# mks0601/ExAvatar_RELEASE

Hardware: NVIDIA H100
Metric: avatar train-step frames/sec (fwd+bwd raster) (higher is better)
Workload: dtype f32

## Files before the change

exavatar_release_b200/csrc/binning.cu:

```cuda
#include <cstdlib>

#include "common.cuh"

namespace b2r {

__global__ void __launch_bounds__(256) scatter_kernel(const B2RScene sc, const Ctx cx, const int first_row) {
  const int i = first_row + blockIdx.x * blockDim.x + threadIdx.x;
  int4 aux = make_int4(0, 0, 0, 0);
  float4 g0 = make_float4(0.f, 0.f, 0.f, 0.f), g1 = g0;
  uint32_t depth_bits = 0u;
  if (i < sc.P) {
    aux = cx.aux[i];
    if (aux.z > 0) {
      const int area = ((aux.y & 0xffff) - (aux.x & 0xffff)) * ((aux.y >> 16) - (aux.x >> 16));
      depth_bits = __float_as_uint(cx.geom[i].g1.z);
      if (area > 32) {
        g0 = reinterpret_cast<const float4*>(cx.geom + i)[0];
        g1 = reinterpret_cast<const float4*>(cx.geom + i)[1];
      }
    }
  }
  const uint64_t cap = cx.dup_capacity;
  const int gx = cx.gx;
  uint32_t* cursor = cx.tile_cursor;
// ... 25 lines not shown
      const int area = ((aux.y & 0xffff) - (aux.x & 0xffff)) * ((aux.y >> 16) - (aux.x >> 16));
      depth_bits = __float_as_uint(cx.geom[i].g1.z);
      if (area > 32) {
        g0 = reinterpret_cast<const float4*>(cx.geom + i)[0];
        g1 = reinterpret_cast<const float4*>(cx.geom + i)[1];
      }
    }
  }
  const int gx = cx.gx;
  const bool no_cull = (sc.flags & B2R_FLAG_NO_TILE_CULL) != 0;
  const int x0 = aux.x & 0xffff, y0 = aux.x >> 16, x1 = aux.y & 0xffff, y1 = aux.y >> 16;
  const uint32_t kept = (uint32_t)aux.w;
  warp_replay_kept_tiles(aux.z > 0, x0, y0, x1, y1, kept, g0.x, g0.y, g0.z, g0.w, g1.x, g1.w, 0u, 0u, no_cull, sc.width,
                         sc.height, gx, s_cnt, [](uint32_t, int, uint32_t, uint32_t) {});
  __syncthreads();
  for (int t = threadIdx.x; t < cx.tiles; t += blockDim.x) {
    const uint32_t c = s_cnt[t];
    if (c) {
      s_base[t] = atomicAdd(cx.tile_cursor + t, c);
      s_cnt[t] = 0u;
    }
  }
  __syncthreads();
  const uint64_t cap = cx.dup_capacity;
  uint2* keys = cx.keys;
  warp_replay_kept_tiles(aux.z > 0, x0, y0, x1, y1, kept, g0.x, g0.y, g0.z, g0.w, g1.x, g1.w, depth_bits, (uint32_t)i,
                         no_cull, sc.width, sc.height, gx, s_cnt, [&](uint32_t rank, int t, uint32_t d, uint32_t id) {
                           const uint32_t pos = s_base[t] + rank;
                           if (pos < cap) keys[pos] = make_uint2(d, id);
                         });
}


__device__ __forceinline__ unsigned match_digit(const uint32_t d, const bool valid) {
  unsigned peers = __ballot_sync(0xffffffffu, valid);
#pragma unroll
  for (int bit = 0; bit < 8; bit++) {
    const bool on = (d >> bit) & 1u;
    const unsigned b = __ballot_sync(0xffffffffu, on);
    peers &= on ? b : ~b;
  }
  return valid ? peers : 0u;
}

template <int CAP, int THREADS>
struct RadixSmem {
  static constexpr int W = THREADS / 32;
  static constexpr size_t bytes = (size_t)CAP * 12 + (size_t)W * 256 * 2 + 64;
};

template <int CAP, int THREADS, bool PAIRS = false>
__device__ __forceinline__ void radix_sort_tile(const uint2* src, uint32_t* dst, const int n, unsigned char* smem_raw,
                                                uint32_t* maxid) {
  constexpr int W = THREADS / 32;
  constexpr int ROWS = CAP / (W * 32);
  static_assert(CAP % (W * 32) == 0, "a warp's share must be whole rows");
  uint32_t* keyA = reinterpret_cast<uint32_t*>(smem_raw);
  uint32_t* keyB = keyA + CAP;
  uint16_t* idxA = reinterpret_cast<uint16_t*>(keyB + CAP);
  uint16_t* idxB = idxA + CAP;
  uint16_t* hist = idxB + CAP;
  uint32_t* misc = reinterpret_cast<uint32_t*>(hist + W * 256);
  const int tid = threadIdx.x, lane = tid & 31, warp = tid >> 5;

  if (tid == 0) { misc[0] = 0u; misc[1] = 0xffffffffu; }
  __syncthreads();
  uint32_t vor = 0u, vand = 0xffffffffu;
  for (int i = tid; i < n; i += THREADS) {
    const uint32_t k = src[i].x;
    keyA[i] = k;
    idxA[i] = (uint16_t)i;
    vor |= k;
    vand &= k;
  }
  vor = __reduce_or_sync(0xffffffffu, vor);
  vand = __reduce_and_sync(0xffffffffu, vand);
  if (lane == 0) { atomicOr(&misc[0], vor); atomicAnd(&misc[1], vand); }
  __syncthreads();
  const uint32_t differ = misc[0] ^ misc[1];

  const int chunk = (((n + W - 1) / W) + 31) & ~31;
  const int c_begin = min(warp * chunk, n), c_end = min(c_begin + chunk, n);
  uint32_t* kin = keyA; uint32_t* kout = keyB;
  uint16_t* iin = idxA; uint16_t* iout = idxB;
  for (int pass = 0; pass < 4; pass++) {
    const int shift = 8 * pass;
    if (((differ >> shift) & 0xffu) == 0u) continue;
    for (int i = tid; i < W * 256; i += THREADS) hist[i] = 0;
    __syncthreads();
    uint16_t* myhist = hist + warp * 256;
    unsigned row_peers[ROWS];
#pragma unroll
    for (int r = 0; r < ROWS; r++) {
      const int base = c_begin + 32 * r;
      row_peers[r] = 0u;
      if (base < c_end) {
        const int i = base + lane;
        const bool valid = i < c_end;
        const uint32_t d = valid ? ((kin[i] >> shift) & 0xffu) : (256u + lane);
        const unsigned peers = match_digit(d, valid);
        row_peers[r] = peers;
        if (valid && (peers & ((1u << lane) - 1u)) == 0u) myhist[d] = (uint16_t)(myhist[d] + __popc(peers));
        __syncwarp();
      }
    }
    __syncthreads();
    constexpr int DPT = THREADS >= 256 ? 1 : 256 / THREADS;
    constexpr int SCAN_THREADS = 256 / DPT;
    uint32_t tot[DPT];
    uint32_t total = 0;
    if (tid < SCAN_THREADS) {
#pragma unroll
      for (int r = 0; r < DPT; r++) {
        const int d = tid * DPT + r;
        uint32_t run = 0;
        for (int w = 0; w < W; w++) {
          const uint32_t t = hist[w * 256 + d];
          hist[w * 256 + d] = (uint16_t)run;
          run += t;
        }
        tot[r] = run;
        total += run;
      }
    }
    uint32_t incl = total;
#pragma unroll
    for (int o = 1; o < 32; o <<= 1) {
      const uint32_t v = __shfl_up_sync(0xffffffffu, incl, o);
      if (lane >= o) incl += v;
    }
    if (tid < SCAN_THREADS && lane == 31) misc[2 + warp] = incl;
    __syncthreads();
    if (tid < SCAN_THREADS) {
      uint32_t base = incl - total;
      for (int w = 0; w < warp; w++) base += misc[2 + w];
#pragma unroll
      for (int r = 0; r < DPT; r++) {
        const int d = tid * DPT + r;
        for (int w = 0; w < W; w++) hist[w * 256 + d] = (uint16_t)(hist[w * 256 + d] + base);
        base += tot[r];
      }
    }
    __syncthreads();
#pragma unroll
    for (int r = 0; r < ROWS; r++) {
      const int base = c_begin + 32 * r;
      if (base < c_end) {
        const int i = base + lane;
        const bool valid = i < c_end;
        const uint32_t k = valid ? kin[i] : 0u;
        const uint32_t d = (k >> shift) & 0xffu;
        const unsigned peers = row_peers[r];
        const unsigned below = peers & ((1u << lane) - 1u);
        uint32_t start = 0;
        if (valid && below == 0u) {
          start = myhist[d];
          myhist[d] = (uint16_t)(start + __popc(peers));
        }
        start = __shfl_sync(0xffffffffu, start, valid ? __ffs(peers) - 1 : lane);
        if (valid) {
          const uint32_t o = start + __popc(below);
          kout[o] = k;
          iout[o] = iin[i];
        }
        __syncwarp();
      }
    }
    __syncthreads();
    { uint32_t* t = kin; kin = kout; kout = t; }
    { uint16_t* t = iin; iin = iout; iout = t; }
  }
  uint32_t* ids = kout;
  uint32_t vmax = 0u;
  for (int i = tid; i < n; i += THREADS) {
    const uint32_t id = src[iin[i]].y;
    ids[i] = id;
    vmax = max(vmax, id);
  }
  vmax = __reduce_max_sync(0xffffffffu, vmax);
  if (lane == 0 && vmax) atomicMax(maxid, vmax);
  __syncthreads();
  for (;;) {
    int changed = 0;
#pragma unroll
    for (int phase = 0; phase < 2; phase++) {
      for (int i = 2 * tid + phase; i + 1 < n; i += 2 * THREADS) {
        if (kin[i] == kin[i + 1]) {
          const uint32_t a = ids[i], b = ids[i + 1];
          if (a > b) { ids[i] = b; ids[i + 1] = a; changed = 1; }
        }
      }
      __syncthreads();
    }
    if (!__syncthreads_or(changed)) break;
  }
  if (PAIRS) {
    uint2* out = const_cast<uint2*>(src);
    for (int i = tid; i < n; i += THREADS) out[i] = make_uint2(kin[i], ids[i]);
  } else {
    for (int i = tid; i < n; i += THREADS) dst[i] = ids[i];
  }
  __syncthreads();
}

constexpr int WSORT_CAP = 1 << SORT_CTA_SHIFT;
constexpr size_t WSORT_BYTES = (size_t)WSORT_CAP * 12 + 256 * 2;

__device__ __forceinline__ void warp_sort_tile(const uint2* __restrict__ src, uint32_t* __restrict__ dst, const int n,
                                               unsigned char* smem_warp, uint32_t* __restrict__ maxid) {
  const int lane = threadIdx.x & 31;
  const unsigned below_mask = (1u << lane) - 1u;
  if (n <= 0) return;
  if (n <= 32) {
    const uint2 kv = lane < n ? src[lane] : make_uint2(0xffffffffu, 0xffffffffu);
    const uint32_t m = __reduce_max_sync(0xffffffffu, lane < n ? kv.y : 0u);
    if (lane == 0) *maxid = m;
    const unsigned long long me = ((unsigned long long)kv.x << 32) | kv.y;
    int rank = 0;
    for (int j = 0; j < n; j++) {
      const unsigned long long o = __shfl_sync(0xffffffffu, me, j);
      rank += (o < me) ? 1 : 0;
    }
    if (lane < n) dst[rank] = kv.y;
    return;
  }
  uint32_t* keyA = reinterpret_cast<uint32_t*>(smem_warp);
  uint32_t* keyB = keyA + WSORT_CAP;
  uint16_t* idxA = reinterpret_cast<uint16_t*>(keyB + WSORT_CAP);
  uint16_t* idxB = idxA + WSORT_CAP;
  uint16_t* hist = idxB + WSORT_CAP;
  uint32_t vor = 0u, vand = 0xffffffffu;
  for (int i = lane; i < n; i += 32) {
    const uint32_t k = src[i].x;
    keyA[i] = k;
    idxA[i] = (uint16_t)i;
    vor |= k;
    vand &= k;
  }
  const uint32_t differ = __reduce_or_sync(0xffffffffu, vor) ^ __reduce_and_sync(0xffffffffu, vand);
  __syncwarp();
  uint32_t* kin = keyA; uint32_t* kout = keyB;
  uint16_t* iin = idxA; uint16_t* iout = idxB;
  for (int pass = 0; pass < 4; pass++) {
    const int shift = 8 * pass;
    if (((differ >> shift) & 0xffu) == 0u) continue;
    reinterpret_cast<uint4*>(hist)[lane] = make_uint4(0u, 0u, 0u, 0u);
    __syncwarp();
    constexpr int CACHED = 8;
    unsigned row_peers[CACHED];
#pragma unroll
    for (int r = 0; r < CACHED; r++) {
      const int base = 32 * r;
      row_peers[r] = 0u;
      if (base < n) {
        const int i = base + lane;
        const bool valid = i < n;
        const uint32_t d = valid ? ((kin[i] >> shift) & 0xffu) : (256u + lane);
        const unsigned peers = match_digit(d, valid);
        row_peers[r] = peers;
        if (valid && (peers & below_mask) == 0u) hist[d] = (uint16_t)(hist[d] + __popc(peers));
        __syncwarp();
      }
    }
    for (int base = 32 * CACHED; base < n; base += 32) {
// ... 16 lines not shown
    uint32_t run = incl - total;
#pragma unroll
    for (int r = 0; r < 8; r++) { hist[8 * lane + r] = (uint16_t)run; run += c[r]; }
    __syncwarp();
    auto place_row = [&](const int base, const bool cached, const unsigned cached_peers) {
        const int i = base + lane;
        const bool valid = i < n;
        const uint32_t k = valid ? kin[i] : 0u;
        const uint32_t d = valid ? ((k >> shift) & 0xffu) : (256u + lane);
        const unsigned peers = cached ? cached_peers : match_digit(d, valid);
        const unsigned below = peers & below_mask;
        uint32_t start = 0;
        if (valid && below == 0u) {
          start = hist[d];
          hist[d] = (uint16_t)(start + __popc(peers));
        }
        start = __shfl_sync(0xffffffffu, start, valid ? __ffs(peers) - 1 : lane);
        if (valid) {
          const uint32_t o = start + __popc(below);
          kout[o] = k;
          iout[o] = iin[i];
        }
        __syncwarp();
    };
#pragma unroll
    for (int r = 0; r < CACHED; r++)
      if (32 * r < n) place_row(32 * r, true, row_peers[r]);
    for (int base = 32 * CACHED; base < n; base += 32) place_row(base, false, 0u);
    { uint32_t* t = kin; kin = kout; kout = t; }
    { uint16_t* t = iin; iin = iout; iout = t; }
  }
  uint32_t* ids = kout;
  uint32_t vmax = 0u;
  for (int i = lane; i < n; i += 32) {
    const uint32_t id = src[iin[i]].y;
    ids[i] = id;
    vmax = max(vmax, id);
  }
  vmax = __reduce_max_sync(0xffffffffu, vmax);
  if (lane == 0) *maxid = vmax;
  __syncwarp();
  for (;;) {
    bool changed = false;
#pragma unroll
    for (int phase = 0; phase < 2; phase++) {
      for (int i = 2 * lane + phase; i + 1 < n; i += 64) {
        if (kin[i] == kin[i + 1]) {
          const uint32_t a = ids[i], b = ids[i + 1];
          if (a > b) { ids[i] = b; ids[i + 1] = a; changed = true; }
        }
      }
      __syncwarp();
    }
    if (!__any_sync(0xffffffffu, changed)) break;
  }
  for (int i = lane; i < n; i += 32) dst[i] = ids[i];
  __syncwarp();
}

template <int CAP, int THREADS>
__global__ void __launch_bounds__(THREADS) sort_mixed_kernel(const Ctx cx) {
  extern __shared__ __align__(16) unsigned char smem_raw[];
  B2R_TRACE_BEGIN();
  const unsigned long long cls = cx.status->reserved[0];
  const int n_large = (int)(cls & 0xffffffffull), n_ge512 = (int)(cls >> 32);
  const int n_chunks = (int)cx.status->reserved[1];
  const int n_cta = n_ge512 - n_large;
  const int n_warp_items = (cx.tiles - n_ge512 + (THREADS / 32) - 1) / (THREADS / 32);
  const int items = n_chunks + n_cta + n_warp_items;
  int last_n = 0;
  for (int b = blockIdx.x; b < items; b += gridDim.x) {
    if (b < n_chunks) {
      int lo = 0, hi = n_large - 1;
      while (lo < hi) {
        const int mid = (lo + hi + 1) >> 1;
        if ((int)cx.chunk_start[mid] <= b) lo = mid; else hi = mid - 1;
      }
      const uint32_t tile = cx.tile_order[lo];
      const uint2 r = cx.ranges[tile];
      const int off = (b - (int)cx.chunk_start[lo]) * SORT_CHUNK;
      const int len = min(SORT_CHUNK, sort_length(cx, (int)tile, r) - off);
      if (len > 1) radix_sort_tile<CAP, THREADS, true>(cx.keys + r.x + off, nullptr, len, smem_raw, cx.tile_maxid + tile);
      else if (len == 1 && threadIdx.x == 0) atomicMax(cx.tile_maxid + tile, cx.keys[r.x + off].y);
      last_n = len;
    } else if (b < n_chunks + n_cta) {
      const uint32_t tile = cx.tile_order[n_large + (b - n_chunks)];
      const uint2 r = cx.ranges[tile];
      const int n = sort_length(cx, (int)tile, r);
      const uint2* src = cx.keys + r.x;
      uint32_t* dst = cx.dup_ids + r.x;
      if (n > 32) {
        radix_sort_tile<CAP, THREADS>(src, dst, n, smem_raw, cx.tile_maxid + tile);
      } else {
        if (threadIdx.x < 32) warp_sort_tile(src, dst, n, smem_raw, cx.tile_maxid + tile);
// ... 105 lines not shown
    launch_tile_scan(quiet, st);
  }
  if (sc.P > 0) {
    ProfScope p(K_SCATTER, st);
    const size_t smem = (size_t)cx.tiles * 8;
    if (cx.tiles <= 2048) {
      cudaFuncSetAttribute(scatter_agg_kernel, cudaFuncAttributeMaxDynamicSharedMemorySize, 96 * 1024);
      launch_k(scatter_agg_kernel, (sc.P + 255) / 256, 256, smem, st, true, sc, cx, 0);
    } else {
      launch_k(scatter_kernel, (sc.P + 255) / 256, 256, 0, st, true, sc, cx, 0);
    }
  }
  launch_sort(cx, st);
  return check_launch();
}

void launch_sort(const Ctx& cx, cudaStream_t st) {
  const int sms = device_sm_count();
  constexpr int ST = 256;
  constexpr size_t cta_bytes = RadixSmem<SORT_SMALL, ST>::bytes, warp_bytes = (ST / 32) * WSORT_BYTES;
  constexpr size_t small_bytes = cta_bytes > warp_bytes ? cta_bytes : warp_bytes;
  cudaFuncSetAttribute(sort_mixed_kernel<SORT_SMALL, ST>, cudaFuncAttributeMaxDynamicSharedMemorySize, (int)small_bytes);
  {
    ProfScope p(K_SORT_SMALL, st);
    launch_k(sort_mixed_kernel<SORT_SMALL, ST>, cx.tiles, ST, small_bytes, st, true, cx);
  }
  {
    ProfScope p(K_SORT_LARGE, st);
    launch_k(merge_chunks_kernel, 2 * sms, 256, 0, st, true, cx);
  }
}


__global__ void __launch_bounds__(256) split_prepare_kernel(const Ctx cx, const Ctx base, const int split,
                                                            int32_t* __restrict__ radii) {
  const int tid = threadIdx.x;
  const float4* gsrc = reinterpret_cast<const float4*>(base.geom);
  float4* gdst = reinterpret_cast<float4*>(cx.geom);
  for (size_t k = (size_t)blockIdx.x * 256 + tid; k < (size_t)split * 3; k += (size_t)gridDim.x * 256) gdst[k] = gsrc[k];
  for (int k = blockIdx.x * 256 + tid; k < split; k += gridDim.x * 256) radii[k] = base.aux[k].z;
  for (int t = blockIdx.x; t < cx.tiles; t += gridDim.x) {
    const uint32_t own = cx.tile_count[t];
    uint32_t s = 0;
    if (own) {
      const uint2 rb = base.ranges[t];
      for (uint32_t k = rb.x; k < rb.y; k += 256)
        s += (uint32_t)__syncthreads_count(k + tid < rb.y && base.dup_ids[k + tid] < (uint32_t)split);
    }
    if (tid == 0) {
      cx.sort_len[t] = own;
      cx.tile_count[t] = own + s;
    }
    __syncthreads();
  }
}

constexpr int SPLIT_CHUNK = 2048;
constexpr int SPLIT_PER = 8;
__global__ void __launch_bounds__(256) split_merge_kernel(const Ctx cx, const Ctx base, const uint32_t* __restrict__ own_ids,
                                                          const int split) {
  __shared__ uint2 other[SPLIT_CHUNK];
  __shared__ uint32_t wtot[8];
  const int tid = threadIdx.x, lane = tid & 31, warp = tid >> 5;
  const uint32_t tile = cx.tile_order[blockIdx.x];
  const uint2 r = cx.ranges[tile];
  const int n = (int)(r.y - r.x);
  if (n == 0) return;
  const int n_own = sort_length(cx, (int)tile, r);
  uint2* keys = cx.keys + r.x;
  for (int i = tid; i < n_own; i += 256) {
    const uint32_t id = own_ids[r.x + i];
    keys[i] = make_uint2(__float_as_uint(cx.geom[id].g1.z), id);
  }
  const uint2 rb = base.ranges[tile];
  int n_base = 0;
  for (uint32_t k0 = rb.x; k0 < rb.y; k0 += 256) {
    const uint32_t k = k0 + tid;
    const uint32_t id = k < rb.y ? base.dup_ids[k] : 0xffffffffu;
    const bool take = id < (uint32_t)split;
    const unsigned b = __ballot_sync(0xffffffffu, take);
    if (lane == 0) wtot[warp] = __popc(b);
    __syncthreads();
    int off = n_base, tot = 0;
    for (int w = 0; w < 8; w++) {
      off += w < warp ? (int)wtot[w] : 0;
      tot += (int)wtot[w];
    }
    off += __popc(b & ((1u << lane) - 1u));
    if (take && n_own + off < n) keys[n_own + off] = make_uint2(__float_as_uint(cx.geom[id].g1.z), id);
    n_base += tot;
    __syncthreads();
  }
  __syncthreads();
  if (n_own + n_base != n) {
    for (int i = tid; i < n; i += 256) cx.dup_ids[r.x + i] = keys[i].y;
    return;
  }
  for (int side = 0; side < 2; side++) {
    const uint2* mine = side ? keys + n_own : keys;
    const uint2* oth = side ? keys : keys + n_own;
    const int n_mine = side ? n_base : n_own, n_oth = side ? n_own : n_base;
    for (int x0 = 0; x0 < n_mine; x0 += 256 * SPLIT_PER) {
      unsigned long long key[SPLIT_PER];
      int rank[SPLIT_PER];
#pragma unroll
      for (int j = 0; j < SPLIT_PER; j++) {
        const int i = x0 + j * 256 + tid;
        const uint2 v = i < n_mine ? mine[i] : make_uint2(0u, 0u);
        key[j] = ((unsigned long long)v.x << 32) | v.y;
        rank[j] = i;
      }
      for (int c0 = 0; c0 < n_oth; c0 += SPLIT_CHUNK) {
        const int len2 = min(SPLIT_CHUNK, n_oth - c0);
        __syncthreads();
        for (int i = tid; i < len2; i += 256) other[i] = oth[c0 + i];
        __syncthreads();
#pragma unroll
        for (int j = 0; j < SPLIT_PER; j++) {
          int l = 0;
          for (int step = SPLIT_CHUNK; step >= 1; step >>= 1) {
            const int probe = l + step;
            if (probe <= len2) {
              const uint2 v = other[probe - 1];
              if ((((unsigned long long)v.x << 32) | v.y) < key[j]) l = probe;
            }
          }
          rank[j] += l;
        }
      }
#pragma unroll
      for (int j = 0; j < SPLIT_PER; j++)
        if (x0 + j * 256 + tid < n_mine) cx.dup_ids[r.x + rank[j]] = (uint32_t)(key[j] & 0xffffffffull);
    }
  }
}

int launch_binning_split(const B2RScene& sc, const Ctx& cx_in, const Ctx& base, uint32_t* own_ids, const int first_row,
                         int32_t* radii, cudaStream_t st) {
  const Ctx& cx = cx_in;
  {
    ProfScope p(K_MISC, st);
    launch_k(split_prepare_kernel, cx.tiles, 256, 0, st, true, cx, base, first_row, radii);
  }
  launch_tile_scan(cx, st, cx.dup_capacity > 0 ? 1 : 0);
  if (sc.P > first_row) {
    ProfScope p(K_SCATTER, st);
    const unsigned grid = (unsigned)((sc.P - first_row + 255) / 256);
    if (cx.tiles <= 2048) {
      cudaFuncSetAttribute(scatter_agg_kernel, cudaFuncAttributeMaxDynamicSharedMemorySize, 96 * 1024);
      launch_k(scatter_agg_kernel, grid, 256, (size_t)cx.tiles * 8, st, true, sc, cx, first_row);
    } else {
      launch_k(scatter_kernel, grid, 256, 0, st, true, sc, cx, first_row);
    }
  }
  Ctx own = cx;
  own.dup_ids = own_ids;
  launch_sort(own, st);
  {
    ProfScope p(K_SORT_LARGE, st);
    launch_k(split_merge_kernel, cx.tiles, 256, 0, st, true, cx, base, own_ids, first_row);
  }
  return check_launch();
}

}
// ... 7 lines not shown
```

exavatar_release_b200/csrc/composite_bwd4.cu:

```cuda
#include "common.cuh"

namespace b2r {

constexpr int B4_THREADS = 64;
constexpr int B4_BATCH = 64;
#ifndef B4_QUEUE_DEPTH
#define B4_QUEUE_DEPTH 16
#endif
#ifndef B4_MIN_BLOCKS
#define B4_MIN_BLOCKS 10
#endif
constexpr int B4_QUEUE = B4_QUEUE_DEPTH;

struct B4Stage {
  float4 a[B4_BATCH];
  float4 b[B4_BATCH];
  float4 c[B4_BATCH];
};
constexpr int B4_GROUP = 4;
constexpr int B4_CQ = 32 + B4_GROUP;
struct B4Compact {
  float4 r[3][B4_CQ];
};
static_assert(B4_QUEUE % B4_GROUP == 0, "phase B runs when whole groups fill the transposition queue");

__device__ __forceinline__ float rcp_approx4(float x) {
  float y;
  asm("rcp.approx.ftz.f32 %0, %1;" : "=f"(y) : "f"(x));
  return y;
}

struct B4Smem {
  B4Stage stage[2];
  B4Compact compact[2];
  float2 tb[2][B4_QUEUE][33];
  float4 qm0[2][B4_QUEUE];
  float4 qm1[2][B4_QUEUE];
  float4 gpix[2][32];
  int warp_max_s[2];
};

template <bool HAS_DA>
__device__ __forceinline__ void bwd4_item(const B2RScene& sc, const Ctx& cx, const B2RBackwardArgs& args,
                                          float* __restrict__ gacc, B4Smem& sm, const int t_pos, const int seg,
                                          const int quad, const int n_multi) {
  B4Stage (&stage)[2] = sm.stage;
  B4Compact (&compact)[2] = sm.compact;
  float2 (&tb)[2][B4_QUEUE][33] = sm.tb;
  float4 (&qm0)[2][B4_QUEUE] = sm.qm0;
  float4 (&qm1)[2][B4_QUEUE] = sm.qm1;
  float4 (&gpix)[2][32] = sm.gpix;
  int (&warp_max_s)[2] = sm.warp_max_s;
  B2R_TRACE_BEGIN();
  const bool multi = t_pos < n_multi;
  const int tile = (int)cx.tile_order[t_pos];
  if (cx.skip_below && cx.tile_maxid[tile] < cx.skip_below) return;
  const int tx = tile % cx.gx, ty = tile / cx.gx;
  const int lane = threadIdx.x & 31, warp = threadIdx.x >> 5;
  const int W = sc.width, H = sc.height;
  const int wx0 = tx * TILE + (quad & 1) * 8, wy0 = ty * TILE + (quad >> 1) * 8 + warp * 4;
  if (wx0 >= W || ty * TILE + (quad >> 1) * 8 >= H) return;
  const int px = wx0 + (lane & 7), py = wy0 + (lane >> 3);
  const bool inside = px < W && py < H;
  const float pxf = (float)px, pyf = (float)py;
  const float rx0 = (float)wx0, ry0 = (float)wy0;
  const float rx1 = fminf((float)(wx0 + 7), (float)(W - 1)), ry1 = fminf((float)(wy0 + 3), (float)(H - 1));
  const size_t N = (size_t)W * H;
  const size_t pix = (size_t)py * W + px;

  const uint2 range = cx.ranges[tile];
  const int n = (int)(range.y - range.x);
  const int lo = multi ? seg * SEG : 0;
  const int hi = multi ? min(n, lo + SEG) : n;
  const uint32_t* ids = cx.dup_ids + range.x + lo;

  const int my_n = inside ? (int)cx.n_contrib[pix] : 0;
  const int my_hi = min(my_n, hi) - lo;
  const bool cont = my_n > hi;
  const float T_final = inside ? cx.final_T[pix] : 0.f;
  const float g_r = inside ? __ldg(args.dL_dcolor + pix) : 0.f;
  const float g_g = inside ? __ldg(args.dL_dcolor + N + pix) : 0.f;
  const float g_b = inside ? __ldg(args.dL_dcolor + 2 * N + pix) : 0.f;
  float g_d = 0.f, g_a = 0.f;
// ... 3 lines not shown
  }
  const float* bgp = cx.bg ? cx.bg : sc.bg;
  const float Tfb = T_final * (__ldg(bgp) * g_r + __ldg(bgp + 1) * g_g + __ldg(bgp + 2) * g_b);
  gpix[warp][lane] = make_float4(g_r, g_g, g_b, g_d);

  const int warp_n = __reduce_max_sync(0xffffffffu, max(my_hi, 0));
  if (lane == 0) warp_max_s[warp] = warp_n;
  __syncthreads();
  const int nmax = max(warp_max_s[0], warp_max_s[1]);
  if (nmax == 0) {
    B2R_TRACE_END(0);
    return;
  }
  const int nb = (nmax + B4_BATCH - 1) / B4_BATCH;

  float T = T_final, B = 0.f;
  if (cont) {
    const int pit = (py - ty * TILE) * TILE + (px - tx * TILE);
    const int nrec = (n + SEG - 1) / SEG;
    const float* rec = cx.ckpt + (size_t)(cx.seg_start[t_pos] + seg) * CK_REC_FLOATS;
    const float* fin = cx.ckpt + (size_t)(cx.seg_start[t_pos] + nrec - 1) * CK_REC_FLOATS;
    const float4 c = __ldg(reinterpret_cast<const float4*>(rec) + pit);
    const float4 f = __ldg(reinterpret_cast<const float4*>(fin) + pit);
    float num = (f.y - c.y) * g_r + (f.z - c.z) * g_g + (f.w - c.w) * g_b;
    if (HAS_DA) {
      const float2 c2 = __ldg(reinterpret_cast<const float2*>(rec + CK_PLANE0) + pit);
      const float2 f2 = __ldg(reinterpret_cast<const float2*>(fin + CK_PLANE0) + pit);
      num += (f2.x - c2.x) * g_d + (f2.y - c2.y) * g_a;
    }
    T = c.x;
    B = __fdividef(num, c.x);
  }
  float la = 0.f, olm = 1.f, lv = 0.f;
  int qpos = 0;
  B4Compact& cw = compact[warp];
  const bool lane0 = lane == 0;
  const unsigned lanes_above = 0xfffffffeu << lane;
  const uint32_t first_grad = args.first_row;

  auto drain = [&](const int count) {
    constexpr int SHARE = 32 / B4_QUEUE;
    constexpr int ROWS = 4 / SHARE;
    static_assert(B4_QUEUE == 8 || B4_QUEUE == 16 || B4_QUEUE == 32, "queue depth");
    __syncwarp();
    const int h = lane & (B4_QUEUE - 1), part = lane / B4_QUEUE;
    const bool live = h < count;
    float Sx = 0.f, Sy = 0.f, Sxx = 0.f, Sxy = 0.f, Syy = 0.f, Sq = 0.f, Sr = 0.f, Sg = 0.f, Sb = 0.f, Sd = 0.f;
    float4 m0 = make_float4(0.f, 0.f, 0.f, 0.f), m1 = make_float4(0.f, 1.f, 0.f, 0.f);
    if (live) {
      m0 = qm0[warp][h];
      m1 = qm1[warp][h];
      const float mx = m0.x - rx0, my = m0.y - ry0;
      float dxs[8];
#pragma unroll
      for (int c = 0; c < 8; c++) dxs[c] = mx - (float)c;
#pragma unroll
      for (int r = 0; r < ROWS; r++) {
        const float dy = my - (float)(part * ROWS + r);
        float Rq = 0.f, Rx = 0.f, Rxx = 0.f;
#pragma unroll
        for (int c = 0; c < 8; c++) {
          const int p = (part * ROWS + r) * 8 + c;
          const float2 t = tb[warp][h][p];
          const float4 g = gpix[warp][p];
          const float hx = t.x * dxs[c];
          Rq += t.x;
          Rx += hx;
          Rxx = fmaf(hx, dxs[c], Rxx);
          Sr = fmaf(t.y, g.x, Sr);
          Sg = fmaf(t.y, g.y, Sg);
          Sb = fmaf(t.y, g.z, Sb);
          if (HAS_DA) Sd = fmaf(t.y, g.w, Sd);
        }
        const float hy = Rq * dy;
        Sq += Rq;
        Sx += Rx;
        Sxx += Rxx;
        Sy += hy;
        Syy = fmaf(hy, dy, Syy);
        Sxy = fmaf(Rx, dy, Sxy);
      }
    }
#pragma unroll
    for (int o = B4_QUEUE; o < 32; o <<= 1) {
      Sx += __shfl_xor_sync(0xffffffffu, Sx, o);
      Sy += __shfl_xor_sync(0xffffffffu, Sy, o);
      Sxx += __shfl_xor_sync(0xffffffffu, Sxx, o);
      Sxy += __shfl_xor_sync(0xffffffffu, Sxy, o);
      Syy += __shfl_xor_sync(0xffffffffu, Syy, o);
      Sq += __shfl_xor_sync(0xffffffffu, Sq, o);
      Sr += __shfl_xor_sync(0xffffffffu, Sr, o);
      Sg += __shfl_xor_sync(0xffffffffu, Sg, o);
      Sb += __shfl_xor_sync(0xffffffffu, Sb, o);
      if (HAS_DA) Sd += __shfl_xor_sync(0xffffffffu, Sd, o);
    }
    const uint32_t gid = __float_as_uint(m1.z) & 0x1fffffffu;
    if (live && part == 0 && gid >= first_grad) {
      float* dst = gacc + (size_t)gid * 12;
      red_add_v4(dst, 2.f * m0.z * Sx + m0.w * Sy, 2.f * m1.x * Sy + m0.w * Sx, Sxx, Sxy);
      red_add_v4(dst + 4, Syy, __fdividef(Sq, m1.y), Sd, 0.f);
      red_add_v4(dst + 8, Sr, Sg, Sb, 0.f);
    }
    __syncwarp();
  };

  const uint32_t id_begin = cx.id_begin, id_span = cx.id_span;
  uint32_t next_id = 0u;
  auto prefetch = [&](int b) {
    const int idx = b * B4_BATCH + threadIdx.x;
    next_id = idx < nmax ? __ldg(ids + idx) : 0u;
  };
  auto issue = [&](int b) {
    B4Stage& s = stage[b & 1];
    const int idx = b * B4_BATCH + threadIdx.x;
    if (idx < nmax) {
      const uint32_t id = next_id;
      if (id - id_begin < id_span) {
        const float4* src = reinterpret_cast<const float4*>(cx.geom + id);
        cp_async16(&s.a[threadIdx.x], src);
        cp_async16(&s.b[threadIdx.x], src + 1);
        cp_async16(&s.c[threadIdx.x], src + 2);
      } else {
        s.a[threadIdx.x] = make_float4(0.f, 0.f, -1.f, 0.f);
        s.b[threadIdx.x] = make_float4(-1.f, 0.f, 0.f, INFINITY);
      }
    }
    cp_async_commit();
  };

  auto replay_group = [&](const int k) {
    float araw[B4_GROUP], vv[B4_GROUP];
    bool valid[B4_GROUP];
#pragma unroll
    for (int u = 0; u < B4_GROUP; u++) {
      const float4 a = cw.r[0][k + u], bb = cw.r[1][k + u], col = cw.r[2][k + u];
      const float dx = a.x - pxf, dy = a.y - pyf;
      const float p2 = a.z * dx * dx + bb.x * dy * dy + a.w * dx * dy;
      araw[u] = bb.y * ex2_approx(p2);
      valid[u] = (__float_as_int(bb.w) < my_hi) && (p2 <= 0.f) && (araw[u] >= K_ALPHA_MIN);
      float v = fmaf(col.z, g_b, fmaf(col.y, g_g, col.x * g_r));
      if (HAS_DA) v += fmaf(bb.z, g_d, g_a);
      vv[u] = v;
      if (lane0) {
        qm0[warp][qpos + u] = a;
        qm1[warp][qpos + u] = make_float4(bb.x, bb.y, col.w, 0.f);
      }
    }
#pragma unroll
    for (int u = 0; u < B4_GROUP; u++) {
      const float ae = valid[u] ? fminf(K_ALPHA_MAX, araw[u]) : 0.f;
      const float om = 1.f - ae;
      const float rcp = rcp_approx4(om);
      const float Tn = T * rcp;
      B = fmaf(la, lv, olm * B);
      const float dLda = fmaf(vv[u] - B, Tn, -Tfb * rcp);
      la = ae; olm = om; lv = vv[u]; T = Tn;
      tb[warp][qpos + u][lane] = make_float2(valid[u] ? araw[u] * dLda : 0.f, ae * Tn);
    }
    qpos += B4_GROUP;
    if (qpos == B4_QUEUE) {
      drain(B4_QUEUE);
      qpos = 0;
    }
  };

  int head = 0, fill = 0;
  prefetch(nb - 1);
  issue(nb - 1);
  if (nb > 1) prefetch(nb - 2);
  for (int b = nb - 1; b >= 0; b--) {
    cp_async_wait<0>();
    __syncthreads();
    if (b > 0) {
      issue(b - 1);
      if (b > 1) prefetch(b - 2);
    }
    const int count = min(B4_BATCH, nmax - b * B4_BATCH);
    const B4Stage& s = stage[b & 1];
    if (warp_n <= b * B4_BATCH) continue;
    for (int c0 = ((count - 1) >> 5) << 5; c0 >= 0; c0 -= 32) {
      const int idx = c0 + lane;
      const int pos = b * B4_BATCH + idx;
      bool hit = false;
      float4 a, bb;
      if (idx < count && pos < warp_n) {
        a = s.a[idx];
        bb = s.b[idx];
        hit = !(region_max_p2(a.x, a.y, a.z, a.w, bb.x, rx0, ry0, rx1, ry1) < bb.w);
      }
      const unsigned mask = __ballot_sync(0xffffffffu, hit);
      if (mask == 0u) continue;
      if (hit) {
        int slot = head + fill + __popc(mask & lanes_above);
        slot -= slot >= B4_CQ ? B4_CQ : 0;
        cw.r[0][slot] = a;
        cw.r[1][slot] = make_float4(bb.x, bb.y, bb.z, __int_as_float(pos));
        cw.r[2][slot] = s.c[idx];
      }
      fill += __popc(mask);
      __syncwarp();
      for (; fill >= B4_GROUP; fill -= B4_GROUP) {
        replay_group(head);
        head = head + B4_GROUP == B4_CQ ? 0 : head + B4_GROUP;
      }
      __syncwarp();
    }
  }
  if (fill > 0) {
    if (lane >= fill && lane < B4_GROUP) {
      cw.r[0][head + lane] = make_float4(0.f, 0.f, 0.f, 0.f);
      cw.r[1][head + lane] = make_float4(0.f, 1.f, 0.f, __int_as_float(0x7fffffff));
      cw.r[2][head + lane] = make_float4(0.f, 0.f, 0.f, 0.f);
    }
    __syncwarp();
    replay_group(head);
  }
  if (qpos > 0) drain(qpos);
  if (threadIdx.x == 0) atomicAdd(reinterpret_cast<unsigned long long*>(&cx.status->consumed_bwd), (unsigned long long)nmax);
  B2R_TRACE_END(nmax);
}

template <bool HAS_DA>
__global__ void __launch_bounds__(B4_THREADS, B4_MIN_BLOCKS) composite_bwd4_kernel(const B2RScene sc, const Ctx cx,
                                                                    const B2RBackwardArgs args, float* __restrict__ gacc) {
  __shared__ B4Smem sm;
  const int n_multi = cx.ckpt ? (int)cx.classes[CLS_N_MULTI] : 0;
  const int total_segs = cx.ckpt ? (int)cx.classes[CLS_TOTAL_SEGS] : 0;
  const int items = 4 * (total_segs + (cx.tiles - n_multi));
  for (int item = blockIdx.x; item < items; item += gridDim.x) {
    const int s_item = item >> 2;
    int t_pos, seg;
    if (s_item < total_segs) {
      const uint2 e = cx.seg_table[s_item];
      t_pos = (int)e.x;
      seg = (int)e.y;
    } else {
      t_pos = n_multi + (s_item - total_segs);
      seg = 0;
    }
    bwd4_item<HAS_DA>(sc, cx, args, gacc, sm, t_pos, seg, item & 3, n_multi);
    __syncthreads();
  }
}

int launch_composite_bwd(const B2RScene& sc, const Ctx& cx, const B2RBackwardArgs& a, float* gacc, cudaStream_t st) {
  if (!(a.flags & B2R_BWD_SCRATCH_ZEROED)) cudaMemsetAsync(gacc, 0, (size_t)(sc.P > 0 ? sc.P : 1) * 12 * sizeof(float), st);
  const uint64_t extra = cx.ckpt ? cx.dup_capacity / SEG : 0;
  const uint64_t bound = 4ull * ((uint64_t)cx.tiles + extra);
  const uint64_t cap = (uint64_t)device_sm_count() * B4_MIN_BLOCKS * 4;
  const unsigned grid = (unsigned)(bound < cap ? bound : cap);
  ProfScope p(K_COMPOSITE_BWD, st);
  if (a.dL_ddepth || a.dL_dalpha)
    launch_k(composite_bwd4_kernel<true>, grid, B4_THREADS, 0, st, false, sc, cx, a, gacc);
  else
    launch_k(composite_bwd4_kernel<false>, grid, B4_THREADS, 0, st, false, sc, cx, a, gacc);
  return check_launch();
}

}

#ifdef B2R_CTA_TRACE
extern "C" int b2r_debug_trace_bwd(unsigned long long* buf) {
// ... 4 lines not shown
```

Baseline: 1904.

## Use min-offset adaptive-width radix passes and merge-path split merge

The block radix sort now takes the min/max key range, subtracts the minimum, and sorts the span in as few passes as possible with up to 10-bit digits. The histogram scan is packed as four u16 counters per thread. The split merge replaces the per-element binary search against shared-memory chunks with a merge-path partition, so each thread merges its own output slice. Gather loops are batched by SPLIT_PER for memory-level parallelism, and the sort kernel gets a min-blocks launch bound. The trade-offs are a larger histogram in shared memory, which may lower occupancy, and a serial per-thread merge loop.

```diff
diff --git a/exavatar_release_b200/csrc/binning.cu b/exavatar_release_b200/csrc/binning.cu
--- a/exavatar_release_b200/csrc/binning.cu
+++ b/exavatar_release_b200/csrc/binning.cu
@@ -81,21 +81,27 @@
 }
 
 
-__device__ __forceinline__ unsigned match_digit(const uint32_t d, const bool valid) {
+template <int MAX_BITS = 8>
+__device__ __forceinline__ unsigned match_digit(const uint32_t d, const bool valid, const int bits = MAX_BITS) {
   unsigned peers = __ballot_sync(0xffffffffu, valid);
 #pragma unroll
-  for (int bit = 0; bit < 8; bit++) {
-    const bool on = (d >> bit) & 1u;
-    const unsigned b = __ballot_sync(0xffffffffu, on);
-    peers &= on ? b : ~b;
+  for (int bit = 0; bit < MAX_BITS; bit++) {
+    if (bit < bits) {
+      const bool on = (d >> bit) & 1u;
+      const unsigned b = __ballot_sync(0xffffffffu, on);
+      peers &= on ? b : ~b;
+    }
   }
   return valid ? peers : 0u;
 }
+
+constexpr int RADIX_BITS = 10;
+constexpr int RADIX_BINS = 1 << RADIX_BITS;
 
 template <int CAP, int THREADS>
 struct RadixSmem {
   static constexpr int W = THREADS / 32;
-  static constexpr size_t bytes = (size_t)CAP * 12 + (size_t)W * 256 * 2 + 64;
+  static constexpr size_t bytes = (size_t)CAP * 12 + (size_t)W * RADIX_BINS * 2 + 64;
 };
 
 template <int CAP, int THREADS, bool PAIRS = false>
@@ -109,35 +115,42 @@
   uint16_t* idxA = reinterpret_cast<uint16_t*>(keyB + CAP);
   uint16_t* idxB = idxA + CAP;
   uint16_t* hist = idxB + CAP;
-  uint32_t* misc = reinterpret_cast<uint32_t*>(hist + W * 256);
+  uint32_t* misc = reinterpret_cast<uint32_t*>(hist + W * RADIX_BINS);
   const int tid = threadIdx.x, lane = tid & 31, warp = tid >> 5;
 
-  if (tid == 0) { misc[0] = 0u; misc[1] = 0xffffffffu; }
-  __syncthreads();
-  uint32_t vor = 0u, vand = 0xffffffffu;
+  if (tid == 0) { misc[0] = 0xffffffffu; misc[1] = 0u; }
+  __syncthreads();
+  uint32_t kmin_t = 0xffffffffu, kmax_t = 0u;
+#pragma unroll 4
   for (int i = tid; i < n; i += THREADS) {
     const uint32_t k = src[i].x;
     keyA[i] = k;
     idxA[i] = (uint16_t)i;
-    vor |= k;
-    vand &= k;
-  }
-  vor = __reduce_or_sync(0xffffffffu, vor);
-  vand = __reduce_and_sync(0xffffffffu, vand);
-  if (lane == 0) { atomicOr(&misc[0], vor); atomicAnd(&misc[1], vand); }
-  __syncthreads();
-  const uint32_t differ = misc[0] ^ misc[1];
+    kmin_t = min(kmin_t, k);
+    kmax_t = max(kmax_t, k);
+  }
+  kmin_t = __reduce_min_sync(0xffffffffu, kmin_t);
+  kmax_t = __reduce_max_sync(0xffffffffu, kmax_t);
+  if (lane == 0) { atomicMin(&misc[0], kmin_t); atomicMax(&misc[1], kmax_t); }
+  __syncthreads();
+  const uint32_t kmin = misc[0];
+  const int span = 32 - __clz(misc[1] - kmin);
+  const int passes = (span + RADIX_BITS - 1) / RADIX_BITS;
+  const int bits = passes ? (span + passes - 1) / passes : 0;
+  const uint32_t mask = (1u << bits) - 1u;
 
   const int chunk = (((n + W - 1) / W) + 31) & ~31;
   const int c_begin = min(warp * chunk, n), c_end = min(c_begin + chunk, n);
   uint32_t* kin = keyA; uint32_t* kout = keyB;
   uint16_t* iin = idxA; uint16_t* iout = idxB;
-  for (int pass = 0; pass < 4; pass++) {
-    const int shift = 8 * pass;
-    if (((differ >> shift) & 0xffu) == 0u) continue;
-    for (int i = tid; i < W * 256; i += THREADS) hist[i] = 0;
+  for (int pass = 0; pass < passes; pass++) {
+    const int shift = bits * pass;
+    const int zshift = max(bits - 3, 0);
+    for (int i = tid; i < (W << zshift); i += THREADS)
+      reinterpret_cast<uint4*>(hist + (i >> zshift) * RADIX_BINS)[i & ((1 << zshift) - 1)] = make_uint4(0u, 0u, 0u, 0u);
+    const bool scans = 4 * tid < (1 << bits);
     __syncthreads();
-    uint16_t* myhist = hist + warp * 256;
+    uint16_t* myhist = hist + warp * RADIX_BINS;
     unsigned row_peers[ROWS];
 #pragma unroll
     for (int r = 0; r < ROWS; r++) {
@@ -146,48 +159,44 @@
       if (base < c_end) {
         const int i = base + lane;
         const bool valid = i < c_end;
-        const uint32_t d = valid ? ((kin[i] >> shift) & 0xffu) : (256u + lane);
-        const unsigned peers = match_digit(d, valid);
+        const uint32_t d = valid ? ((kin[i] - kmin) >> shift) & mask : 0u;
+        const unsigned peers = match_digit<RADIX_BITS>(d, valid, bits);
         row_peers[r] = peers;
         if (valid && (peers & ((1u << lane) - 1u)) == 0u) myhist[d] = (uint16_t)(myhist[d] + __popc(peers));
         __syncwarp();
       }
     }
     __syncthreads();
-    constexpr int DPT = THREADS >= 256 ? 1 : 256 / THREADS;
-    constexpr int SCAN_THREADS = 256 / DPT;
-    uint32_t tot[DPT];
-    uint32_t total = 0;
-    if (tid < SCAN_THREADS) {
-#pragma unroll
-      for (int r = 0; r < DPT; r++) {
-        const int d = tid * DPT + r;
-        uint32_t run = 0;
-        for (int w = 0; w < W; w++) {
-          const uint32_t t = hist[w * 256 + d];
-          hist[w * 256 + d] = (uint16_t)run;
-          run += t;
-        }
-        tot[r] = run;
-        total += run;
-      }
-    }
+    static_assert(RADIX_BINS == 4 * THREADS && CAP < 65536, "four u16 counters per thread and warp");
+    uint2* hist4 = reinterpret_cast<uint2*>(hist) + tid;
+    uint2 run = make_uint2(0u, 0u);
+    if (scans) {
+#pragma unroll
+      for (int w = 0; w < W; w++) {
+        const uint2 c = hist4[w * THREADS];
+        hist4[w * THREADS] = run;
+        run.x += c.x;
+        run.y += c.y;
+      }
+    }
+    const uint32_t t0 = run.x & 0xffffu, t1 = run.x >> 16, t2 = run.y & 0xffffu;
+    const uint32_t total = t0 + t1 + t2 + (run.y >> 16);
     uint32_t incl = total;
 #pragma unroll
     for (int o = 1; o < 32; o <<= 1) {
       const uint32_t v = __shfl_up_sync(0xffffffffu, incl, o);
       if (lane >= o) incl += v;
     }
-    if (tid < SCAN_THREADS && lane == 31) misc[2 + warp] = incl;
+    if (lane == 31) misc[2 + warp] = incl;
     __syncthreads();
-    if (tid < SCAN_THREADS) {
+    if (scans) {
       uint32_t base = incl - total;
       for (int w = 0; w < warp; w++) base += misc[2 + w];
-#pragma unroll
-      for (int r = 0; r < DPT; r++) {
-        const int d = tid * DPT + r;
-        for (int w = 0; w < W; w++) hist[w * 256 + d] = (uint16_t)(hist[w * 256 + d] + base);
-        base += tot[r];
+      const uint2 off = make_uint2(base | ((base + t0) << 16), (base + t0 + t1) | ((base + t0 + t1 + t2) << 16));
+#pragma unroll
+      for (int w = 0; w < W; w++) {
+        const uint2 c = hist4[w * THREADS];
+        hist4[w * THREADS] = make_uint2(c.x + off.x, c.y + off.y);
       }
     }
     __syncthreads();
@@ -198,7 +207,7 @@
         const int i = base + lane;
         const bool valid = i < c_end;
         const uint32_t k = valid ? kin[i] : 0u;
-        const uint32_t d = (k >> shift) & 0xffu;
+        const uint32_t d = ((k - kmin) >> shift) & mask;
         const unsigned peers = row_peers[r];
         const unsigned below = peers & ((1u << lane) - 1u);
         uint32_t start = 0;
@@ -221,6 +230,7 @@
   }
   uint32_t* ids = kout;
   uint32_t vmax = 0u;
+#pragma unroll 4
   for (int i = tid; i < n; i += THREADS) {
     const uint32_t id = src[iin[i]].y;
     ids[i] = id;
@@ -279,6 +289,7 @@
   uint16_t* idxB = idxA + WSORT_CAP;
   uint16_t* hist = idxB + WSORT_CAP;
   uint32_t vor = 0u, vand = 0xffffffffu;
+#pragma unroll 4
   for (int i = lane; i < n; i += 32) {
     const uint32_t k = src[i].x;
     keyA[i] = k;
@@ -361,6 +372,7 @@
   }
   uint32_t* ids = kout;
   uint32_t vmax = 0u;
+#pragma unroll 4
   for (int i = lane; i < n; i += 32) {
     const uint32_t id = src[iin[i]].y;
     ids[i] = id;
@@ -388,7 +400,7 @@
 }
 
 template <int CAP, int THREADS>
-__global__ void __launch_bounds__(THREADS) sort_mixed_kernel(const Ctx cx) {
+__global__ void __launch_bounds__(THREADS, 4) sort_mixed_kernel(const Ctx cx) {
   extern __shared__ __align__(16) unsigned char smem_raw[];
   B2R_TRACE_BEGIN();
   const unsigned long long cls = cx.status->reserved[0];
@@ -560,6 +572,8 @@
 }
 
 
+constexpr int SPLIT_PER = 8;
+
 __global__ void __launch_bounds__(256) split_prepare_kernel(const Ctx cx, const Ctx base, const int split,
                                                             int32_t* __restrict__ radii) {
   const int tid = threadIdx.x;
@@ -567,13 +581,25 @@
   float4* gdst = reinterpret_cast<float4*>(cx.geom);
   for (size_t k = (size_t)blockIdx.x * 256 + tid; k < (size_t)split * 3; k += (size_t)gridDim.x * 256) gdst[k] = gsrc[k];
   for (int k = blockIdx.x * 256 + tid; k < split; k += gridDim.x * 256) radii[k] = base.aux[k].z;
+  __shared__ uint32_t wsum[8];
   for (int t = blockIdx.x; t < cx.tiles; t += gridDim.x) {
     const uint32_t own = cx.tile_count[t];
     uint32_t s = 0;
     if (own) {
       const uint2 rb = base.ranges[t];
-      for (uint32_t k = rb.x; k < rb.y; k += 256)
-        s += (uint32_t)__syncthreads_count(k + tid < rb.y && base.dup_ids[k + tid] < (uint32_t)split);
+      uint32_t c = 0;
+      for (uint32_t k0 = rb.x; k0 < rb.y; k0 += 256 * SPLIT_PER) {
+#pragma unroll
+        for (int j = 0; j < SPLIT_PER; j++) {
+          const uint32_t k = k0 + j * 256 + tid;
+          c += (k < rb.y && base.dup_ids[k] < (uint32_t)split) ? 1u : 0u;
+        }
+      }
+      c = __reduce_add_sync(0xffffffffu, c);
+      if ((tid & 31) == 0) wsum[tid >> 5] = c;
+      __syncthreads();
+#pragma unroll
+      for (int w = 0; w < 8; w++) s += wsum[w];
     }
     if (tid == 0) {
       cx.sort_len[t] = own;
@@ -583,11 +609,8 @@
   }
 }
 
-constexpr int SPLIT_CHUNK = 2048;
-constexpr int SPLIT_PER = 8;
 __global__ void __launch_bounds__(256) split_merge_kernel(const Ctx cx, const Ctx base, const uint32_t* __restrict__ own_ids,
                                                           const int split) {
-  __shared__ uint2 other[SPLIT_CHUNK];
   __shared__ uint32_t wtot[8];
   const int tid = threadIdx.x, lane = tid & 31, warp = tid >> 5;
   const uint32_t tile = cx.tile_order[blockIdx.x];
@@ -596,26 +619,54 @@
   if (n == 0) return;
   const int n_own = sort_length(cx, (int)tile, r);
   uint2* keys = cx.keys + r.x;
-  for (int i = tid; i < n_own; i += 256) {
-    const uint32_t id = own_ids[r.x + i];
-    keys[i] = make_uint2(__float_as_uint(cx.geom[id].g1.z), id);
+  for (int i0 = 0; i0 < n_own; i0 += 256 * SPLIT_PER) {
+    uint32_t id[SPLIT_PER];
+    float z[SPLIT_PER];
+#pragma unroll
+    for (int j = 0; j < SPLIT_PER; j++) {
+      const int i = i0 + j * 256 + tid;
+      id[j] = i < n_own ? own_ids[r.x + i] : 0u;
+    }
+#pragma unroll
+    for (int j = 0; j < SPLIT_PER; j++) z[j] = i0 + j * 256 + tid < n_own ? cx.geom[id[j]].g1.z : 0.f;
+#pragma unroll
+    for (int j = 0; j < SPLIT_PER; j++) {
+      const int i = i0 + j * 256 + tid;
+      if (i < n_own) keys[i] = make_uint2(__float_as_uint(z[j]), id[j]);
+    }
   }
   const uint2 rb = base.ranges[tile];
   int n_base = 0;
-  for (uint32_t k0 = rb.x; k0 < rb.y; k0 += 256) {
-    const uint32_t k = k0 + tid;
-    const uint32_t id = k < rb.y ? base.dup_ids[k] : 0xffffffffu;
-    const bool take = id < (uint32_t)split;
-    const unsigned b = __ballot_sync(0xffffffffu, take);
-    if (lane == 0) wtot[warp] = __popc(b);
+  for (uint32_t k0 = rb.x; k0 < rb.y; k0 += 256 * SPLIT_PER) {
+    uint32_t id[SPLIT_PER];
+    unsigned b[SPLIT_PER];
+    int wcount = 0;
+#pragma unroll
+    for (int j = 0; j < SPLIT_PER; j++) {
+      const uint32_t k = k0 + (warp * SPLIT_PER + j) * 32 + lane;
+      id[j] = k < rb.y ? base.dup_ids[k] : 0xffffffffu;
+    }
+#pragma unroll
+    for (int j = 0; j < SPLIT_PER; j++) {
+      b[j] = __ballot_sync(0xffffffffu, id[j] < (uint32_t)split);
+      wcount += __popc(b[j]);
+    }
+    if (lane == 0) wtot[warp] = wcount;
     __syncthreads();
     int off = n_base, tot = 0;
     for (int w = 0; w < 8; w++) {
       off += w < warp ? (int)wtot[w] : 0;
       tot += (int)wtot[w];
     }
-    off += __popc(b & ((1u << lane) - 1u));
-    if (take && n_own + off < n) keys[n_own + off] = make_uint2(__float_as_uint(cx.geom[id].g1.z), id);
+    float z[SPLIT_PER];
+#pragma unroll
+    for (int j = 0; j < SPLIT_PER; j++) z[j] = id[j] < (uint32_t)split ? cx.geom[id[j]].g1.z : 0.f;
+#pragma unroll
+    for (int j = 0; j < SPLIT_PER; j++) {
+      const int o = off + __popc(b[j] & ((1u << lane) - 1u));
+      if (id[j] < (uint32_t)split && n_own + o < n) keys[n_own + o] = make_uint2(__float_as_uint(z[j]), id[j]);
+      off += __popc(b[j]);
+    }
     n_base += tot;
     __syncthreads();
   }
@@ -624,41 +675,26 @@
     for (int i = tid; i < n; i += 256) cx.dup_ids[r.x + i] = keys[i].y;
     return;
   }
-  for (int side = 0; side < 2; side++) {
-    const uint2* mine = side ? keys + n_own : keys;
-    const uint2* oth = side ? keys : keys + n_own;
-    const int n_mine = side ? n_base : n_own, n_oth = side ? n_own : n_base;
-    for (int x0 = 0; x0 < n_mine; x0 += 256 * SPLIT_PER) {
-      unsigned long long key[SPLIT_PER];
-      int rank[SPLIT_PER];
-#pragma unroll
-      for (int j = 0; j < SPLIT_PER; j++) {
-        const int i = x0 + j * 256 + tid;
-        const uint2 v = i < n_mine ? mine[i] : make_uint2(0u, 0u);
-        key[j] = ((unsigned long long)v.x << 32) | v.y;
-        rank[j] = i;
-      }
-      for (int c0 = 0; c0 < n_oth; c0 += SPLIT_CHUNK) {
-        const int len2 = min(SPLIT_CHUNK, n_oth - c0);
-        __syncthreads();
-        for (int i = tid; i < len2; i += 256) other[i] = oth[c0 + i];
-        __syncthreads();
-#pragma unroll
-        for (int j = 0; j < SPLIT_PER; j++) {
-          int l = 0;
-          for (int step = SPLIT_CHUNK; step >= 1; step >>= 1) {
-            const int probe = l + step;
-            if (probe <= len2) {
-              const uint2 v = other[probe - 1];
-              if ((((unsigned long long)v.x << 32) | v.y) < key[j]) l = probe;
-            }
-          }
-          rank[j] += l;
-        }
-      }
-#pragma unroll
-      for (int j = 0; j < SPLIT_PER; j++)
-        if (x0 + j * 256 + tid < n_mine) cx.dup_ids[r.x + rank[j]] = (uint32_t)(key[j] & 0xffffffffull);
+  const uint2* own = keys;
+  const uint2* oth = keys + n_own;
+  const int d0 = (int)(((long long)n * tid) / 256), d1 = (int)(((long long)n * (tid + 1)) / 256);
+  if (d0 == d1) return;
+  auto key64 = [](const uint2 v) { return ((unsigned long long)v.x << 32) | v.y; };
+  int lo = max(0, d0 - n_base), hi = min(d0, n_own);
+  while (lo < hi) {
+    const int mid = (lo + hi) >> 1;
+    if (key64(own[mid]) < key64(oth[d0 - mid - 1])) lo = mid + 1; else hi = mid;
+  }
+  int i = lo, j = d0 - lo;
+  unsigned long long a = i < n_own ? key64(own[i]) : ~0ull, c = j < n_base ? key64(oth[j]) : ~0ull;
+  uint32_t* out = cx.dup_ids + r.x;
+  for (int d = d0; d < d1; d++) {
+    if (a < c) {
+      out[d] = (uint32_t)a;
+      a = ++i < n_own ? key64(own[i]) : ~0ull;
+    } else {
+      out[d] = (uint32_t)c;
+      c = ++j < n_base ? key64(oth[j]) : ~0ull;
     }
   }
 }
```

Result: no change. 1902 (median of 6 runs) (-0.1%).

## Read drain metadata from compact queue, skip drains with no gradient rows

Applied to the files above, without the earlier changes.

Removes the separate per-warp metadata queues (qm0/qm1) written by lane 0 during replay. Drain now reads Gaussian parameters directly from the compaction ring, whose size grows to 32+queue depth so that drains never wrap. Drain exits early when no entry in the batch needs a gradient (gid < first_row), and accumulator initialisation is folded into the first term. It also adds an optional half-batch staging mode where two threads split the three cp.async loads per entry, and re-reads class counts inside the item loop. The cost is a larger compact buffer and reliance on the ring-alignment invariants.

```diff
diff --git a/exavatar_release_b200/csrc/composite_bwd4.cu b/exavatar_release_b200/csrc/composite_bwd4.cu
--- a/exavatar_release_b200/csrc/composite_bwd4.cu
+++ b/exavatar_release_b200/csrc/composite_bwd4.cu
@@ -3,7 +3,11 @@
 namespace b2r {
 
 constexpr int B4_THREADS = 64;
-constexpr int B4_BATCH = 64;
+#ifndef B4_BATCH_SIZE
+#define B4_BATCH_SIZE 64
+#endif
+constexpr int B4_BATCH = B4_BATCH_SIZE;
+static_assert(B4_BATCH == B4_THREADS || 2 * B4_BATCH == B4_THREADS, "one or two gathering threads per staged entry");
 #ifndef B4_QUEUE_DEPTH
 #define B4_QUEUE_DEPTH 16
 #endif
@@ -18,11 +22,12 @@
   float4 c[B4_BATCH];
 };
 constexpr int B4_GROUP = 4;
-constexpr int B4_CQ = 32 + B4_GROUP;
+constexpr int B4_CQ = 32 + B4_QUEUE;
 struct B4Compact {
   float4 r[3][B4_CQ];
 };
 static_assert(B4_QUEUE % B4_GROUP == 0, "phase B runs when whole groups fill the transposition queue");
+static_assert(32 % B4_QUEUE == 0 && B4_CQ % B4_GROUP == 0, "drains and groups never straddle the queue's wrap");
 
 __device__ __forceinline__ float rcp_approx4(float x) {
   float y;
@@ -34,8 +39,6 @@
   B4Stage stage[2];
   B4Compact compact[2];
   float2 tb[2][B4_QUEUE][33];
-  float4 qm0[2][B4_QUEUE];
-  float4 qm1[2][B4_QUEUE];
   float4 gpix[2][32];
   int warp_max_s[2];
 };
@@ -47,8 +50,6 @@
   B4Stage (&stage)[2] = sm.stage;
   B4Compact (&compact)[2] = sm.compact;
   float2 (&tb)[2][B4_QUEUE][33] = sm.tb;
-  float4 (&qm0)[2][B4_QUEUE] = sm.qm0;
-  float4 (&qm1)[2][B4_QUEUE] = sm.qm1;
   float4 (&gpix)[2][32] = sm.gpix;
   int (&warp_max_s)[2] = sm.warp_max_s;
   B2R_TRACE_BEGIN();
@@ -118,53 +119,58 @@
     B = __fdividef(num, c.x);
   }
   float la = 0.f, olm = 1.f, lv = 0.f;
-  int qpos = 0;
   B4Compact& cw = compact[warp];
-  const bool lane0 = lane == 0;
   const unsigned lanes_above = 0xfffffffeu << lane;
   const uint32_t first_grad = args.first_row;
 
-  auto drain = [&](const int count) {
+  auto drain = [&](const int base, const int count) {
     constexpr int SHARE = 32 / B4_QUEUE;
     constexpr int ROWS = 4 / SHARE;
     static_assert(B4_QUEUE == 8 || B4_QUEUE == 16 || B4_QUEUE == 32, "queue depth");
     __syncwarp();
     const int h = lane & (B4_QUEUE - 1), part = lane / B4_QUEUE;
     const bool live = h < count;
+    const uint32_t gid = live ? __float_as_uint(cw.r[2][base + h].w) & 0x1fffffffu : 0u;
+    if (!__any_sync(0xffffffffu, live && gid >= first_grad)) {
+      __syncwarp();
+      return;
+    }
     float Sx = 0.f, Sy = 0.f, Sxx = 0.f, Sxy = 0.f, Syy = 0.f, Sq = 0.f, Sr = 0.f, Sg = 0.f, Sb = 0.f, Sd = 0.f;
     float4 m0 = make_float4(0.f, 0.f, 0.f, 0.f), m1 = make_float4(0.f, 1.f, 0.f, 0.f);
     if (live) {
-      m0 = qm0[warp][h];
-      m1 = qm1[warp][h];
+      m0 = cw.r[0][base + h];
+      m1 = cw.r[1][base + h];
       const float mx = m0.x - rx0, my = m0.y - ry0;
       float dxs[8];
 #pragma unroll
       for (int c = 0; c < 8; c++) dxs[c] = mx - (float)c;
+      auto add = [](float& s, const float x, const bool first) { s = first ? x : s + x; };
+      auto mad = [](float& s, const float x, const float y, const bool first) { s = first ? x * y : fmaf(x, y, s); };
 #pragma unroll
       for (int r = 0; r < ROWS; r++) {
         const float dy = my - (float)(part * ROWS + r);
-        float Rq = 0.f, Rx = 0.f, Rxx = 0.f;
+        float Rq, Rx, Rxx;
 #pragma unroll
         for (int c = 0; c < 8; c++) {
           const int p = (part * ROWS + r) * 8 + c;
           const float2 t = tb[warp][h][p];
           const float4 g = gpix[warp][p];
           const float hx = t.x * dxs[c];
-          Rq += t.x;
-          Rx += hx;
-          Rxx = fmaf(hx, dxs[c], Rxx);
-          Sr = fmaf(t.y, g.x, Sr);
-          Sg = fmaf(t.y, g.y, Sg);
-          Sb = fmaf(t.y, g.z, Sb);
-          if (HAS_DA) Sd = fmaf(t.y, g.w, Sd);
+          add(Rq, t.x, c == 0);
+          add(Rx, hx, c == 0);
+          mad(Rxx, hx, dxs[c], c == 0);
+          mad(Sr, t.y, g.x, r + c == 0);
+          mad(Sg, t.y, g.y, r + c == 0);
+          mad(Sb, t.y, g.z, r + c == 0);
+          if (HAS_DA) mad(Sd, t.y, g.w, r + c == 0);
         }
         const float hy = Rq * dy;
-        Sq += Rq;
-        Sx += Rx;
-        Sxx += Rxx;
-        Sy += hy;
-        Syy = fmaf(hy, dy, Syy);
-        Sxy = fmaf(Rx, dy, Sxy);
+        add(Sq, Rq, r == 0);
+        add(Sx, Rx, r == 0);
+        add(Sxx, Rxx, r == 0);
+        add(Sy, hy, r == 0);
+        mad(Syy, hy, dy, r == 0);
+        mad(Sxy, Rx, dy, r == 0);
       }
     }
 #pragma unroll
@@ -180,7 +186,6 @@
       Sb += __shfl_xor_sync(0xffffffffu, Sb, o);
       if (HAS_DA) Sd += __shfl_xor_sync(0xffffffffu, Sd, o);
     }
-    const uint32_t gid = __float_as_uint(m1.z) & 0x1fffffffu;
     if (live && part == 0 && gid >= first_grad) {
       float* dst = gacc + (size_t)gid * 12;
       red_add_v4(dst, 2.f * m0.z * Sx + m0.w * Sy, 2.f * m1.x * Sy + m0.w * Sx, Sxx, Sxy);
@@ -192,23 +197,27 @@
 
   const uint32_t id_begin = cx.id_begin, id_span = cx.id_span;
   uint32_t next_id = 0u;
+  const int ge = B4_BATCH == B4_THREADS ? (int)threadIdx.x : threadIdx.x & (B4_BATCH - 1);
+  const bool g_ab = B4_BATCH == B4_THREADS || threadIdx.x < B4_BATCH, g_c = B4_BATCH == B4_THREADS || !g_ab;
   auto prefetch = [&](int b) {
-    const int idx = b * B4_BATCH + threadIdx.x;
+    const int idx = b * B4_BATCH + ge;
     next_id = idx < nmax ? __ldg(ids + idx) : 0u;
   };
   auto issue = [&](int b) {
     B4Stage& s = stage[b & 1];
-    const int idx = b * B4_BATCH + threadIdx.x;
+    const int idx = b * B4_BATCH + ge;
     if (idx < nmax) {
       const uint32_t id = next_id;
       if (id - id_begin < id_span) {
         const float4* src = reinterpret_cast<const float4*>(cx.geom + id);
-        cp_async16(&s.a[threadIdx.x], src);
-        cp_async16(&s.b[threadIdx.x], src + 1);
-        cp_async16(&s.c[threadIdx.x], src + 2);
-      } else {
-        s.a[threadIdx.x] = make_float4(0.f, 0.f, -1.f, 0.f);
-        s.b[threadIdx.x] = make_float4(-1.f, 0.f, 0.f, INFINITY);
+        if (g_ab) {
+          cp_async16(&s.a[ge], src);
+          cp_async16(&s.b[ge], src + 1);
+        }
+        if (g_c) cp_async16(&s.c[ge], src + 2);
+      } else if (g_ab) {
+        s.a[ge] = make_float4(0.f, 0.f, -1.f, 0.f);
+        s.b[ge] = make_float4(-1.f, 0.f, 0.f, INFINITY);
       }
     }
     cp_async_commit();
@@ -216,38 +225,31 @@
 
   auto replay_group = [&](const int k) {
     float araw[B4_GROUP], vv[B4_GROUP];
-    bool valid[B4_GROUP];
 #pragma unroll
     for (int u = 0; u < B4_GROUP; u++) {
       const float4 a = cw.r[0][k + u], bb = cw.r[1][k + u], col = cw.r[2][k + u];
       const float dx = a.x - pxf, dy = a.y - pyf;
       const float p2 = a.z * dx * dx + bb.x * dy * dy + a.w * dx * dy;
-      araw[u] = bb.y * ex2_approx(p2);
-      valid[u] = (__float_as_int(bb.w) < my_hi) && (p2 <= 0.f) && (araw[u] >= K_ALPHA_MIN);
+      const float al = bb.y * ex2_approx(p2);
+      const bool valid = (__float_as_int(bb.w) < my_hi) && (p2 <= 0.f) && (al >= K_ALPHA_MIN);
+      araw[u] = valid ? al : 0.f;
       float v = fmaf(col.z, g_b, fmaf(col.y, g_g, col.x * g_r));
       if (HAS_DA) v += fmaf(bb.z, g_d, g_a);
       vv[u] = v;
-      if (lane0) {
-        qm0[warp][qpos + u] = a;
-        qm1[warp][qpos + u] = make_float4(bb.x, bb.y, col.w, 0.f);
-      }
-    }
+    }
+    const int row = k & (B4_QUEUE - 1);
 #pragma unroll
     for (int u = 0; u < B4_GROUP; u++) {
-      const float ae = valid[u] ? fminf(K_ALPHA_MAX, araw[u]) : 0.f;
+      const float ae = fminf(K_ALPHA_MAX, araw[u]);
       const float om = 1.f - ae;
       const float rcp = rcp_approx4(om);
       const float Tn = T * rcp;
       B = fmaf(la, lv, olm * B);
       const float dLda = fmaf(vv[u] - B, Tn, -Tfb * rcp);
       la = ae; olm = om; lv = vv[u]; T = Tn;
-      tb[warp][qpos + u][lane] = make_float2(valid[u] ? araw[u] * dLda : 0.f, ae * Tn);
-    }
-    qpos += B4_GROUP;
-    if (qpos == B4_QUEUE) {
-      drain(B4_QUEUE);
-      qpos = 0;
-    }
+      tb[warp][row + u][lane] = make_float2(araw[u] * dLda, ae * Tn);
+    }
+    if (row + B4_GROUP == B4_QUEUE) drain(k - row, B4_QUEUE);
   };
 
   int head = 0, fill = 0;
@@ -300,8 +302,9 @@
     }
     __syncwarp();
     replay_group(head);
-  }
-  if (qpos > 0) drain(qpos);
+    head = head + B4_GROUP == B4_CQ ? 0 : head + B4_GROUP;
+  }
+  if (head & (B4_QUEUE - 1)) drain(head & ~(B4_QUEUE - 1), head & (B4_QUEUE - 1));
   if (threadIdx.x == 0) atomicAdd(reinterpret_cast<unsigned long long*>(&cx.status->consumed_bwd), (unsigned long long)nmax);
   B2R_TRACE_END(nmax);
 }
@@ -310,10 +313,10 @@
 __global__ void __launch_bounds__(B4_THREADS, B4_MIN_BLOCKS) composite_bwd4_kernel(const B2RScene sc, const Ctx cx,
                                                                     const B2RBackwardArgs args, float* __restrict__ gacc) {
   __shared__ B4Smem sm;
-  const int n_multi = cx.ckpt ? (int)cx.classes[CLS_N_MULTI] : 0;
-  const int total_segs = cx.ckpt ? (int)cx.classes[CLS_TOTAL_SEGS] : 0;
-  const int items = 4 * (total_segs + (cx.tiles - n_multi));
-  for (int item = blockIdx.x; item < items; item += gridDim.x) {
+  for (int item = blockIdx.x;; item += gridDim.x) {
+    const int n_multi = cx.ckpt ? (int)cx.classes[CLS_N_MULTI] : 0;
+    const int total_segs = cx.ckpt ? (int)cx.classes[CLS_TOTAL_SEGS] : 0;
+    if (item >= 4 * (total_segs + (cx.tiles - n_multi))) break;
     const int s_item = item >> 2;
     int t_pos, seg;
     if (s_item < total_segs) {
```

Measured after the change: 1902 before, 1958 after, median of 6. 2.9% higher.
